# sd196821/QuadSim

Measured on AMD Instinct MI355X. Metric: env-steps/sec at N parallel envs (1/2/4/8 GPU); per-step state L2 err vs NumPy ref, higher is better.
Workload: dtype f32

## Files before the change

quadsim_amd/csrc/step_kernels.hpp:

```cpp
#pragma once

namespace {

#ifndef QS_BLOCK
#define QS_BLOCK 256
#endif
constexpr int kBlock = QS_BLOCK;
#ifndef QS_PREP_MAX_TILES
#define QS_PREP_MAX_TILES 1365
#endif
constexpr int64_t kPrepMaxTiles = QS_PREP_MAX_TILES;
#ifndef QS_SPLIT_MAX_ENVS
#define QS_SPLIT_MAX_ENVS 131072
#endif
constexpr int64_t kSplitMaxEnvs = QS_SPLIT_MAX_ENVS;

struct StepArgs {
    float *st;
    float *par;
    const float *actions;
    float *obs;
    float *reward;
    uint8_t *done;
    uint8_t *flags;
    float *term_obs;
    float *term_state;
    float *slab;
    int64_t n;
    int64_t tile0, tile_end;
    int64_t dbg_shift;
    int64_t io_env0, io_n;
    int64_t T;
    uint64_t step_idx;
    unsigned long long *ctr;
    uint64_t gid0;
    EnvConst C;
    RandCfg rc;
    Par par_nom;
    int auto_reset;
    int randomise;
    float nominal_obs[12];
    const float *init;
    unsigned *owner;
    unsigned *err;
    unsigned long long *stamps;
    unsigned long long stamp_cap, stamp_tiles;
};

__device__ __forceinline__ void load_env(const float *__restrict__ st, int64_t tile, int lane, Env &e)
{
    const float *b = st + tile * (int64_t)(kRecWords * kTile) + lane;
#pragma unroll
    for (int i = 0; i < 13; ++i) e.sc[i] = b[(F_SC + i) * kTile];
#pragma unroll
    for (int i = 0; i < 13; ++i) e.st[i] = b[(F_ST + i) * kTile];
#pragma unroll
    for (int i = 0; i < 4; ++i) e.uc[i] = b[(F_UC + i) * kTile];
#pragma unroll
    for (int i = 0; i < 4; ++i) e.ut[i] = b[(F_UT + i) * kTile];
#pragma unroll
    for (int i = 0; i < 4; ++i) e.qd[i] = b[(F_QD + i) * kTile];
    e.ls = b[F_LS * kTile];
    e.t = b[F_T * kTile];
}

__device__ __forceinline__ void load_env_or_nominal(const StepArgs &A, int64_t tile, int lane, bool active, Env &e)
{
    if (active) load_env(A.st, tile, lane, e);
    else { nominal_init(e.sc, e.st); for (int i = 0; i < 4; ++i) { e.uc[i] = 0.0f; e.ut[i] = 0.0f; e.qd[i] = i == 0; } e.ls = 0.0f; e.t = 0.0f; }
}

__device__ __forceinline__ void store_env(float *__restrict__ st, int64_t tile, int lane, const Env &e)
{
    float *b = st + tile * (int64_t)(kRecWords * kTile) + lane;
#pragma unroll
    for (int i = 0; i < 13; ++i) QS_ST(&b[(F_SC + i) * kTile], e.sc[i]);
#pragma unroll
    for (int i = 0; i < 13; ++i) QS_ST(&b[(F_ST + i) * kTile], e.st[i]);
#pragma unroll
    for (int i = 0; i < 4; ++i) QS_ST(&b[(F_UC + i) * kTile], e.uc[i]);
#pragma unroll
    for (int i = 0; i < 4; ++i) QS_ST(&b[(F_UT + i) * kTile], e.ut[i]);
#pragma unroll
    for (int i = 0; i < 4; ++i) QS_ST(&b[(F_QD + i) * kTile], e.qd[i]);
    QS_ST(&b[F_LS * kTile], e.ls);
    QS_ST(&b[F_T * kTile], e.t);
}

__device__ __forceinline__ Par load_par(const float *__restrict__ par, int64_t tile, int lane)
{
    const float *b = par + tile * (int64_t)(kParWords * kTile) + lane;
    Par P;
    P.m = b[0]; P.Ixx = b[kTile]; P.Iyy = b[2 * kTile]; P.Izz = b[3 * kTile];
    return P;
}

__device__ __forceinline__ void store_par(float *__restrict__ par, int64_t tile, int lane, const Par &P)
{
    float *b = par + tile * (int64_t)(kParWords * kTile) + lane;
    b[0] = P.m; b[kTile] = P.Ixx; b[2 * kTile] = P.Iyy; b[3 * kTile] = P.Izz;
}

struct TileLane { int lane; int64_t tile, env; bool active; };
__device__ __forceinline__ TileLane tile_lane(int64_t n)
{
    const int lane = threadIdx.x & (kTile - 1);
    const int64_t tile = (int64_t)blockIdx.x * (kBlock / kTile) + (threadIdx.x >> 6);
    const int64_t env = tile * kTile + lane;
    return {lane, tile, env, env < n};
}

__device__ __forceinline__ void store_obs(float *__restrict__ obs, int64_t env, const float o[12])
{
    typedef float f4 __attribute__((ext_vector_type(4)));
    f4 *p = reinterpret_cast<f4 *>(obs + env * 12);
    QS_SO(&p[0], (f4{o[0], o[1], o[2], o[3]}));
    QS_SO(&p[1], (f4{o[4], o[5], o[6], o[7]}));
    QS_SO(&p[2], (f4{o[8], o[9], o[10], o[11]}));
}

__device__ __forceinline__ void store_obs_cached(float *__restrict__ obs, int64_t env, const float o[12])
{
    float4 *p = reinterpret_cast<float4 *>(obs + env * 12);
    p[0] = make_float4(o[0], o[1], o[2], o[3]);
    p[1] = make_float4(o[4], o[5], o[6], o[7]);
    p[2] = make_float4(o[8], o[9], o[10], o[11]);
}

__device__ __forceinline__ uint64_t step_counter_begin(const StepArgs &A, int64_t tile) { return A.ctr[tile]; }
__device__ __forceinline__ uint64_t step_counter_begin_vmem(const StepArgs &A, int64_t tile)
{
    int zero;
    asm("v_mov_b32 %0, 0" : "=v"(zero));
    return A.ctr[tile + zero];
}
__device__ __forceinline__ void step_counter_end(const StepArgs &A, int64_t tile, int lane, uint64_t k)
{
    if (lane == 0) A.ctr[tile] = k + (uint64_t)A.T;
}

constexpr unsigned kUnowned = 0xffffffffu;
__device__ __forceinline__ unsigned chain_owner_request(const StepArgs &A, int64_t tile)
{
    const unsigned *p = A.owner ? A.owner + tile : reinterpret_cast<const unsigned *>(A.ctr + tile);
    const unsigned v = __hip_atomic_load(p, __ATOMIC_RELAXED, __HIP_MEMORY_SCOPE_AGENT);
    return A.owner ? v : kUnowned;
}

__device__ __forceinline__ bool chain_owner_mismatch(const StepArgs &A, int64_t tile, int lane, unsigned own)
{
    const unsigned xcc = __builtin_amdgcn_s_getreg((3 << 11) | (0 << 6) | 20) & 15u;
    if (own == kUnowned) {
        unsigned seen = kUnowned;
        if (lane == 0) {
            unsigned expect = kUnowned;
            __hip_atomic_compare_exchange_strong(&A.owner[tile], &expect, xcc, __ATOMIC_RELAXED, __ATOMIC_RELAXED, __HIP_MEMORY_SCOPE_AGENT);
            seen = expect;
        }
        own = __builtin_amdgcn_readfirstlane(seen);
        if (own == kUnowned) return false;
    }
    if (own != xcc) {
        if (lane == 0) __hip_atomic_fetch_or(A.err, 1u, __ATOMIC_RELAXED, __HIP_MEMORY_SCOPE_SYSTEM);
        return true;
    }
    return false;
}

__device__ __forceinline__ bool chain_tile_misplaced(const StepArgs &A, int64_t tile, int lane)
{
    if (!A.owner) return false;
    return chain_owner_mismatch(A, tile, lane, chain_owner_request(A, tile));
}

__device__ __forceinline__ int64_t launch_tile(const StepArgs &A, int64_t b)
{
    const int64_t nt = A.tile_end - A.tile0;
    b += A.dbg_shift;
    b -= (b >= nt) ? nt : 0;
    return A.tile0 + b;
}

template <bool PARAMS, int RMODE>
__device__ __forceinline__ void maybe_reset(Env &e, Par &P, const StepArgs &A, int64_t env, uint64_t k, float obs[12], unsigned flags,
                                            bool &done, bool write_term);

template <int INTEG, bool PARAMS, int RMODE>
__device__ __forceinline__ void step_and_maybe_reset(Env &e, Par &P, const float a[4], const StepArgs &A, int64_t env,
                                                     uint64_t k, float obs[12], float &reward, unsigned &flags,
                                                     bool &done, bool write_term)
{
    env_step<INTEG>(e, a, P, A.C, obs, reward, flags);
    maybe_reset<PARAMS, RMODE>(e, P, A, env, k, obs, flags, done, write_term);
}

template <bool PARAMS, int RMODE>
__device__ __forceinline__ void maybe_reset(Env &e, Par &P, const StepArgs &A, int64_t env, uint64_t k, float obs[12], unsigned flags,
                                            bool &done, bool write_term)
{
    done = (flags & (FLAG_OVERLIMIT | FLAG_OVERTIME)) != 0;
    if (done && A.auto_reset) {
        if (write_term && A.term_obs) store_obs(A.term_obs, env - A.io_env0, obs);
        if (write_term && A.term_state) {
            float *ts = A.term_state + (env - A.io_env0) * 26;
#pragma unroll
            for (int i = 0; i < 13; ++i) { ts[i] = e.sc[i]; ts[13 + i] = e.st[i]; }
        }
        if (RMODE == 0) {
            nominal_init(e.sc, e.st);
#pragma unroll
            for (int i = 0; i < 4; ++i) { e.uc[i] = 0.0f; e.ut[i] = 0.0f; }
            e.ls = 0.0f;
            e.t = 0.0f;
#pragma unroll
            for (int i = 0; i < 12; ++i) obs[i] = A.nominal_obs[i];
        } else if (RMODE == 3) {
            float ic[13], it[13];
            const float *src = A.init + env * 26;
#pragma unroll
            for (int i = 0; i < 13; ++i) { ic[i] = src[i]; it[i] = src[13 + i]; }
            env_reset<false>(e, ic, it, obs);
        } else {
            float ic[13], it[13];
            Par Pn;
            random_init<RMODE == 2>(A.rc, STREAM_AUTORESET, A.gid0 + (uint64_t)env, k + 1, ic, it, Pn);
            if (PARAMS && RMODE == 2) P = Pn;
            env_reset<true>(e, ic, it, obs);
        }
    }
}

template <int INTEG, bool PARAMS, int RMODE>
__global__ __launch_bounds__(kBlock) void k_env(StepArgs A)
{
    const int lane = threadIdx.x & (kTile - 1);
    const int64_t wg_tile = (int64_t)blockIdx.x * (kBlock / kTile) + (threadIdx.x >> 6);
    if (wg_tile >= A.tile_end - A.tile0) return;
    const int64_t tile = launch_tile(A, wg_tile);
    const int64_t env = tile * kTile + lane;
    if (env >= A.n) return;
    if (chain_tile_misplaced(A, tile, lane)) return;
    const int64_t io = env - A.io_env0;
    QS_ASSERT(io >= 0 && io < A.io_n);
    const uint64_t k0 = step_counter_begin_vmem(A, tile);
    float4 av_next = make_float4(0.0f, 0.0f, 0.0f, 0.0f);
    if (A.actions) av_next = reinterpret_cast<const float4 *>(A.actions)[io];
    Env e;
    load_env(A.st, tile, lane, e);
    Par P = A.par_nom;
    if (PARAMS) P = load_par(A.par, tile, lane);
#pragma clang loop unroll(disable)
    for (int64_t t = 0; t < A.T; ++t) {
        const uint64_t k = k0 + (uint64_t)t;
        const int64_t o = t * A.io_n + io;
        float a[4];
        if (A.actions) {
            const float4 av = av_next;
            if (t + 1 < A.T) av_next = reinterpret_cast<const float4 *>(A.actions)[o + A.io_n];
            a[0] = av.x; a[1] = av.y; a[2] = av.z; a[3] = av.w;
        } else {
            random_action(A.rc.seed, A.gid0 + (uint64_t)env, k, a);
        }
        float obs[12], reward;
        unsigned flags;
        bool done;
        step_and_maybe_reset<INTEG, PARAMS, RMODE>(e, P, a, A, env, k, obs, reward, flags, done, true);
        if (A.slab) {
            float2 *row = reinterpret_cast<float2 *>(A.slab + o * 14);
#pragma unroll
            for (int i = 0; i < 6; ++i) row[i] = make_float2(obs[2 * i], obs[2 * i + 1]);
            row[6] = make_float2(reward, done ? 1.0f : 0.0f);
        } else {
            store_obs(A.obs, o, obs);
            QS_SO(&A.reward[o], reward);
            QS_SO(&A.done[o], (uint8_t)(done ? 1 : 0));
        }
        if (A.flags) QS_SO(&A.flags[o], (uint8_t)flags);
    }
    store_env(A.st, tile, lane, e);
    if (PARAMS && RMODE == 2) store_par(A.par, tile, lane, P);
    step_counter_end(A, tile, lane, k0);
}

constexpr int split_waves(int rmode, int prep) { return (prep == 2 && (rmode == 1 || rmode == 2)) ? 3 : 2; }


constexpr bool split_prep(int rmode, int prep) { return split_waves(rmode, prep) == 3; }
constexpr bool split_draw(int rmode, int prep) { return (rmode == 1 || rmode == 2) && !split_prep(rmode, prep); }
template <int RMODE, int PREP>
struct SplitLds {
    float tgt[13][kTile];
    float rst[split_prep(RMODE, PREP) ? 29 : 0][kTile];
    uint4 phx[split_draw(RMODE, PREP) ? 2 : 0][2][kTile];
    unsigned char done[kTile], limt[kTile];
    __device__ __forceinline__ Par reset_par(int lane) const { return Par{rst[25][lane], rst[26][lane], rst[27][lane], rst[28][lane]}; }
};

__device__ __forceinline__ void chaser_load(const float *b, float sc[13], float uc[4], float &ls, float &tt)
{
#pragma unroll
    for (int i = 0; i < 13; ++i) sc[i] = b[(F_SC + i) * kTile];
#pragma unroll
    for (int i = 0; i < 4; ++i) uc[i] = b[(F_UC + i) * kTile];
    ls = b[F_LS * kTile];
    tt = b[F_T * kTile];
}

__device__ __forceinline__ void chaser_store(float *bw, const float sc[13], const float uc[4], float ls, float tt)
{
#pragma unroll
    for (int i = 0; i < 13; ++i) QS_ST(&bw[(F_SC + i) * kTile], sc[i]);
#pragma unroll
    for (int i = 0; i < 4; ++i) QS_ST(&bw[(F_UC + i) * kTile], uc[i]);
    QS_ST(&bw[F_LS * kTile], ls);
    QS_ST(&bw[F_T * kTile], tt);
}

template <int RMODE, int PREP>
__device__ __forceinline__ bool chaser_score(SplitLds<RMODE, PREP> &L, int lane, const float sc[13], const float a[4], float tt, float &ls,
                                             const EnvConst &C, int auto_reset, bool lim_c, float obs[12], float &reward,
                                             unsigned &flags, bool &done)
{
    float st[13];
#pragma unroll
    for (int i = 0; i < 13; ++i) st[i] = L.tgt[i][lane];
    const bool lim_t = L.limt[lane] != 0;
    rel_obs(sc, st, obs);
    score_step(obs, a, sc[2], tt, ls, C, lim_c, lim_t, reward, flags);
    done = (flags & (FLAG_OVERLIMIT | FLAG_OVERTIME)) != 0;
    const bool rs = done && auto_reset;
    L.done[lane] = rs ? 1 : 0;
    return rs;
}

__device__ __forceinline__ void store_term_half(float *term_state, bool active, int64_t io, int half, const float s[13])
{
    if (term_state && active) {
        float *ts = term_state + io * 26 + 13 * half;
#pragma unroll
        for (int i = 0; i < 13; ++i) ts[i] = s[i];
    }
}

template <bool PARAMS, int RMODE, int PREP>
__device__ __forceinline__ void chaser_reset(const SplitLds<RMODE, PREP> &L, const StepArgs &A, int64_t env, bool active, int lane, int64_t t,
                                             float sc[13], float uc[4], float &ls, float &tt, Par &P, float obs[12])
{
    float ic[13], it[13];
    if (RMODE == 0) {
        nominal_init(ic, it);
#pragma unroll
        for (int i = 0; i < 12; ++i) obs[i] = A.nominal_obs[i];
    } else if (RMODE == 3) {
        const float *src = A.init + (active ? env : 0) * 26;
#pragma unroll
        for (int i = 0; i < 13; ++i) { ic[i] = src[i]; it[i] = src[13 + i]; }
        rel_obs<false>(ic, it, obs);
    } else {
        if constexpr (split_prep(RMODE, PREP)) {
#pragma unroll
            for (int i = 0; i < 13; ++i) ic[i] = L.rst[i][lane];
#pragma unroll
            for (int i = 0; i < 12; ++i) obs[i] = L.rst[13 + i][lane];
            if (PARAMS && RMODE == 2) P = L.reset_par(lane);
        } else {
            const uint4 w0 = L.phx[t & 1][0][lane], w1 = RMODE == 2 ? L.phx[t & 1][1][lane] : make_uint4(0, 0, 0, 0);
            Par Pn;
            random_init_apply<RMODE == 2>(A.rc, w0, w1, ic, it, Pn);
            if (PARAMS && RMODE == 2) P = Pn;
            rel_obs<true>(ic, it, obs);
        }
    }
#pragma unroll
    for (int i = 0; i < 13; ++i) sc[i] = ic[i];
#pragma unroll
    for (int i = 0; i < 4; ++i) uc[i] = 0.0f;
    ls = 0.0f;
    tt = 0.0f;
}

__device__ __forceinline__ void target_load(const float *b, float st[13], float ut[4], float qd[4])
{
#pragma unroll
    for (int i = 0; i < 13; ++i) st[i] = b[(F_ST + i) * kTile];
#pragma unroll
    for (int i = 0; i < 4; ++i) ut[i] = b[(F_UT + i) * kTile];
#pragma unroll
    for (int i = 0; i < 4; ++i) qd[i] = b[(F_QD + i) * kTile];
}

__device__ __forceinline__ void target_store(float *bw, const float st[13], const float ut[4], const float qd[4])
{
#pragma unroll
    for (int i = 0; i < 13; ++i) QS_ST(&bw[(F_ST + i) * kTile], st[i]);
#pragma unroll
    for (int i = 0; i < 4; ++i) QS_ST(&bw[(F_UT + i) * kTile], ut[i]);
#pragma unroll
    for (int i = 0; i < 4; ++i) QS_ST(&bw[(F_QD + i) * kTile], qd[i]);
}

template <int RMODE, int PREP>
__device__ __forceinline__ void target_publish(SplitLds<RMODE, PREP> &L, const StepArgs &A, int64_t env, int lane, uint64_t k, int64_t t,
                                               const float st[13], bool lim_t, uint4 &w0, uint4 &w1)
{
#pragma unroll
    for (int i = 0; i < 13; ++i) L.tgt[i][lane] = st[i];
    L.limt[lane] = lim_t ? 1 : 0;
    w0 = make_uint4(0, 0, 0, 0);
    w1 = w0;
    if constexpr (split_draw(RMODE, PREP)) {
        random_init_words<RMODE == 2>(A.rc, STREAM_AUTORESET, A.gid0 + (uint64_t)env, k + 1, w0, w1);
        L.phx[t & 1][0][lane] = w0;
        if (RMODE == 2) L.phx[t & 1][1][lane] = w1;
    }
}

__device__ __forceinline__ void target_command(const EnvConst &C, float qd[4], const float pre[13], float m, float ut[4])
{
    const float pdes[3] = {10.0f, -50.0f, 5.0f};
    const float vdes[3] = {C.vdes_x, 0.0f, 0.0f};
    const float dv[3] = {0.0f, 0.0f, 0.0f};
    float u_t[4];
    target_control(C.kind, pdes, vdes, qd, 0.0f, pre, dv, m, u_t);
    u_limit(u_t, m * kG, ut);
}

template <bool PARAMS, int RMODE, int PREP>
__device__ __forceinline__ void target_reset(const SplitLds<RMODE, PREP> &L, const StepArgs &A, int64_t env, bool active, int lane,
                                             const uint4 &w0, const uint4 &w1, float st[13], float ut[4], Par &P)
{
    float ic[13], it[13];
    if (RMODE == 3) {
        const float *src = A.init + (active ? env : 0) * 26;
#pragma unroll
        for (int i = 0; i < 13; ++i) it[i] = src[13 + i];
    } else {
        nominal_init(ic, it);
        if (PARAMS && RMODE == 2) {
            if constexpr (split_prep(RMODE, PREP)) {
                P = L.reset_par(lane);
            } else {
                random_init_apply<true>(A.rc, w0, w1, ic, it, P);
                nominal_init(ic, it);
            }
        }
    }
#pragma unroll
    for (int i = 0; i < 13; ++i) st[i] = it[i];
#pragma unroll
    for (int i = 0; i < 4; ++i) ut[i] = 0.0f;
}

template <bool PARAMS, int RMODE, int PREP>
__device__ __forceinline__ void prep_publish(SplitLds<RMODE, PREP> &L, const RandCfg &rc, int lane, const uint4 &w0, const uint4 &w1)
{
    float ic[13], it_[13], robs[12];
    Par Pn;
    random_init_apply<RMODE == 2>(rc, w0, w1, ic, it_, Pn);
    rel_obs<true>(ic, it_, robs);
#pragma unroll
    for (int i = 0; i < 13; ++i) L.rst[i][lane] = ic[i];
#pragma unroll
    for (int i = 0; i < 12; ++i) L.rst[13 + i][lane] = robs[i];
    if (PARAMS && RMODE == 2) {
        L.rst[25][lane] = Pn.m; L.rst[26][lane] = Pn.Ixx; L.rst[27][lane] = Pn.Iyy; L.rst[28][lane] = Pn.Izz;
    }
}

constexpr int kResWords = 8;
constexpr unsigned long long kResPtrMask = (1ull << 48) - 1;
enum { RES_STEP = 0, RES_EXIT = 1, RES_IDLE = 2, RES_SKIP = 3 };
constexpr int kResWin = 32;
constexpr int kResWinSlots = 16;

struct ResArgs {
    const unsigned long long *ring;
    unsigned long long *rseq;
    unsigned *wcnt;
    unsigned *fin;
    unsigned long long *h_prog;
    unsigned long long *h_fin;
    unsigned long long seq0;
    unsigned long long base;
    unsigned long long stop_seq;
    unsigned long long slots_mask;
    unsigned long long idle_ticks;
    unsigned lane_tiles;
};

struct ResDesc {
    const float *actions;
    float *obs, *reward;
    uint8_t *done, *flags;
    float *term_obs, *term_state;
};

__device__ __forceinline__ unsigned long long res_request(const ResArgs &R, unsigned long long s, int lane)
{
    return __hip_atomic_load(R.ring + (s & R.slots_mask) * kResWords + (lane & 7), __ATOMIC_RELAXED, __HIP_MEMORY_SCOPE_SYSTEM);
}

__device__ __forceinline__ bool res_fresh(unsigned long long w, unsigned long long s, int lane)
{
    bool ok = (w >> 48) == (s & 0xffffull);
    if ((lane & 7) == 7) ok = ok && (unsigned)w == (unsigned)(s >> 16);
    return __all(ok);
}

__device__ __forceinline__ unsigned long long res_word(unsigned long long w, int i)
{
    const unsigned lo = (unsigned)__builtin_amdgcn_readlane((int)(unsigned)w, i);
    const unsigned hi = (unsigned)__builtin_amdgcn_readlane((int)(unsigned)(w >> 32), i);
    return (((unsigned long long)hi << 32) | lo) & kResPtrMask;
}

__device__ __forceinline__ int res_resolve(const ResArgs &R, unsigned long long s, int lane, unsigned long long w, ResDesc &D)
{
    if (!res_fresh(w, s, lane)) {
        const unsigned long long t0 = __builtin_amdgcn_s_memrealtime();
        for (;;) {
            __builtin_amdgcn_s_sleep(4);
            w = res_request(R, s, lane);
            if (res_fresh(w, s, lane)) break;
            if (__builtin_amdgcn_s_memrealtime() - t0 > R.idle_ticks) return RES_IDLE;
        }
    }
    D.actions = (const float *)res_word(w, 0);
    D.obs = (float *)res_word(w, 1);
    D.reward = (float *)res_word(w, 2);
    D.done = (uint8_t *)res_word(w, 3);
    D.flags = (uint8_t *)res_word(w, 4);
    D.term_obs = (float *)res_word(w, 5);
    D.term_state = (float *)res_word(w, 6);
    return ((res_word(w, 7) >> 32) & 0xff) == 0 ? RES_STEP : RES_EXIT;
}

__device__ __forceinline__ float4 res_action(const float *actions, int64_t io, int64_t io_n)
{
    typedef unsigned u4 __attribute__((ext_vector_type(4)));
    const __amdgpu_buffer_rsrc_t r = __builtin_amdgcn_make_buffer_rsrc((void *)actions, (short)0, (int)(io_n * 16), 0x00020000);
    const u4 v = __builtin_amdgcn_raw_buffer_load_b128(r, (int)(io * 16), 0, 17);
    return make_float4(__uint_as_float(v.x), __uint_as_float(v.y), __uint_as_float(v.z), __uint_as_float(v.w));
}

__device__ __forceinline__ unsigned res_report(const ResArgs &R, unsigned long long s, int64_t tile, int lane)
{
    const unsigned long long x = s - R.base + (unsigned long long)(tile % kResWin) + 1;
    if (x % kResWin != 0) return ~0u;
    unsigned old = 0;
    if (lane == 0) old = __hip_atomic_fetch_add(R.wcnt + (x / kResWin) % kResWinSlots, 1u, __ATOMIC_RELAXED, __HIP_MEMORY_SCOPE_AGENT);
    return old;
}

__device__ __forceinline__ void res_report_done(const ResArgs &R, unsigned old, unsigned long long s, int64_t tile, int lane)
{
    if (old == ~0u || lane != 0 || (old + 1) % R.lane_tiles != 0) return;
    const unsigned long long x = s - R.base + (unsigned long long)(tile % kResWin) + 1;
    __hip_atomic_store(R.h_prog, R.base + x - kResWin + 1, __ATOMIC_RELAXED, __HIP_MEMORY_SCOPE_SYSTEM);
}

template <int INTEG, bool PARAMS, int RMODE, int PREP>
__global__ __launch_bounds__(3 * kTile) void k_env_resident(StepArgs A, ResArgs R)
{
    __shared__ SplitLds<RMODE, PREP> L;
    __shared__ int s_cmd[2];
    __shared__ unsigned long long s_tsp[2];
    const int lane = threadIdx.x & (kTile - 1);
    const int role = threadIdx.x >> 6;
    const int64_t tile = launch_tile(A, blockIdx.x);
    const int64_t env = tile * kTile + lane;
    bool active = env < A.n;
    const int64_t io = env - A.io_env0;
    QS_ASSERT(tile < A.tile_end && (!active || (io >= 0 && io < A.io_n)));
    const uint64_t k0 = step_counter_begin_vmem(A, tile);
    unsigned long long seq = 0;
    int cmd = RES_STEP;
    ResDesc D{};
    {
        if (role == 0) {
            seq = R.seq0 ? R.seq0 : R.rseq[tile];
            seq = ((unsigned long long)__builtin_amdgcn_readfirstlane((int)(unsigned)(seq >> 32)) << 32) |
                  (unsigned)__builtin_amdgcn_readfirstlane((int)(unsigned)seq);
            cmd = seq >= R.stop_seq ? RES_SKIP : res_resolve(R, seq, lane, res_request(R, seq, lane), D);
            if (cmd == RES_STEP) res_report_done(R, res_report(R, seq, tile, lane), seq, tile, lane);
            if (lane == 0) { s_cmd[0] = cmd; s_tsp[0] = (unsigned long long)D.term_state; }
        }
        __syncthreads();
        cmd = s_cmd[0];
    }
    QS_STAMP_DECL;
    QS_STAMP_AT(0);
    const float *b = A.st + tile * (int64_t)(kRecWords * kTile) + lane;
    float *bw = A.st + tile * (int64_t)(kRecWords * kTile) + lane;
    Par P = A.par_nom;
    if (PARAMS) P = load_par(A.par, tile, lane);
    if (role == 0) {
        __builtin_amdgcn_s_setprio(3);
        float sc[13], uc[4], ls, tt;
        chaser_load(b, sc, uc, ls, tt);
        float4 av_next = make_float4(0.0f, 0.0f, 0.0f, 0.0f);
        if (cmd == RES_STEP && active) av_next = res_action(D.actions, io, A.io_n);
#if defined(QS_STAMP) && QS_STAMP + 0 < 2
        asm volatile("s_waitcnt vmcnt(1)" ::: "memory");
#endif
        QS_STAMP_AT(1);
        int64_t t = 0;
#pragma clang loop unroll(disable)
        for (; cmd == RES_STEP; ++t) {
            const int64_t o = io;
            const unsigned long long wn = res_request(R, seq + t + 1, lane);
            tt += 1.0f;
            const bool lim_c = drone_advance<INTEG>(sc, uc, P, A.C.dt);
            float a[4];
            ResDesc Dn{};
            unsigned rep = ~0u;
            const float4 av = av_next;
            const int cmdn = res_resolve(R, seq + t + 1, lane, wn, Dn);
            if (cmdn == RES_STEP) {
                if (active) av_next = res_action(Dn.actions, io, A.io_n);
                rep = res_report(R, seq + t + 1, tile, lane);
            }
            if (lane == 0) { s_cmd[(t + 1) & 1] = cmdn; s_tsp[(t + 1) & 1] = (unsigned long long)Dn.term_state; }
            a[0] = av.x; a[1] = av.y; a[2] = av.z; a[3] = av.w;
            float u_c[4];
            chaser_command(a, P.m, u_c);
            u_limit(u_c, P.m * kG, uc);
            QS_STAMP_AT(2);
            __syncthreads();
            QS_STAMP_AT(3);
            float obs[12], reward;
            unsigned flags;
            bool done;
            const bool rs = chaser_score(L, lane, sc, a, tt, ls, A.C, A.auto_reset, lim_c, obs, reward, flags, done);
            QS_STAMP_AT(4);
            __syncthreads();
            QS_STAMP_AT(5);
            if (rs) {
                if (D.term_obs && active) store_obs(D.term_obs, io, obs);
                store_term_half(D.term_state, active, io, 0, sc);
                chaser_reset<PARAMS>(L, A, env, active, lane, t, sc, uc, ls, tt, P, obs);
            }
            QS_STAMP_AT(6);
            if (active) {
                store_obs(D.obs, o, obs);
                QS_SO(&D.reward[o], reward);
                QS_SO(&D.done[o], (uint8_t)(done ? 1 : 0));
                if (D.flags) QS_SO(&D.flags[o], (uint8_t)flags);
            }
            res_report_done(R, rep, seq + t + 1, tile, lane);
            D = Dn;
            cmd = cmdn;
        }
        if (t > 0) {
            if (active) {
                chaser_store(bw, sc, uc, ls, tt);
                if (PARAMS && RMODE == 2) store_par(A.par, tile, lane, P);
            }
        }
        {
            if (cmd != RES_SKIP && lane == 0) {
                if (t > 0) A.ctr[tile] = k0 + (uint64_t)t;
                R.rseq[tile] = seq + (unsigned long long)t + (cmd == RES_EXIT ? 1 : 0);
                if (cmd == RES_EXIT) {
                    const unsigned old = __hip_atomic_fetch_add(R.fin, 1u, __ATOMIC_RELAXED, __HIP_MEMORY_SCOPE_AGENT);
                    if (old + 1 == R.lane_tiles)
                        __hip_atomic_store(R.h_fin, seq + (unsigned long long)t + 1, __ATOMIC_RELAXED, __HIP_MEMORY_SCOPE_SYSTEM);
                }
            }
        }
#if defined(QS_STAMP) && QS_STAMP + 0 < 2
        asm volatile("s_waitcnt vmcnt(0)" ::: "memory");
#endif
        QS_STAMP_AT(7);
        QS_STAMP_FLUSH();
    } else if (role == 1) {
        float st[13], ut[4], qd[4];
        target_load(b, st, ut, qd);
#if defined(QS_STAMP) && QS_STAMP + 0 < 2
        asm volatile("s_waitcnt vmcnt(0)" ::: "memory");
#endif
        QS_STAMP_AT(1);
        int64_t t = 0;
#pragma clang loop unroll(disable)
        for (; cmd == RES_STEP; ++t) {
            float pre[13];
#pragma unroll
            for (int i = 0; i < 13; ++i) pre[i] = st[i];
            const bool lim_t = drone_advance<INTEG>(st, ut, P, A.C.dt);
            uint4 w0, w1;
            target_publish(L, A, env, lane, k0 + (uint64_t)t, t, st, lim_t, w0, w1);
            QS_STAMP_AT(2);
            __syncthreads();
            QS_STAMP_AT(3);
            float *const term_state = (float *)s_tsp[t & 1];
            target_command(A.C, qd, pre, P.m, ut);
            QS_STAMP_AT(4);
            __syncthreads();
            QS_STAMP_AT(5);
            if (L.done[lane]) {
                store_term_half(term_state, active, io, 1, st);
                target_reset<PARAMS>(L, A, env, active, lane, w0, w1, st, ut, P);
            }
            cmd = s_cmd[(t + 1) & 1];
        }
        if (active && t > 0) target_store(bw, st, ut, qd);
        QS_STAMP_AT(6);
        QS_STAMP_FLUSH();
    } else if constexpr (split_prep(RMODE, PREP)) {
        int64_t t = 0;
#pragma clang loop unroll(disable)
        for (; cmd == RES_STEP; ++t) {
            uint4 w0, w1 = make_uint4(0, 0, 0, 0);
            random_init_words<RMODE == 2>(A.rc, STREAM_AUTORESET, A.gid0 + (uint64_t)env, k0 + (uint64_t)t + 1, w0, w1);
            __syncthreads();
            prep_publish<PARAMS>(L, A.rc, lane, w0, w1);
            __syncthreads();
            cmd = s_cmd[(t + 1) & 1];
        }
    }
}

template <int INTEG, bool PARAMS, int RMODE, int PREP>
__global__ __launch_bounds__(3 * kTile) void k_env_split(StepArgs A)
{
    __shared__ SplitLds<RMODE, PREP> L;
    const int lane = threadIdx.x & (kTile - 1);
    const int role = threadIdx.x >> 6;
    const int64_t tile = launch_tile(A, blockIdx.x);
    const int64_t env = tile * kTile + lane;
    bool active = env < A.n;
    const int64_t io = env - A.io_env0;
    QS_ASSERT(tile < A.tile_end && (!active || (io >= 0 && io < A.io_n)));
    const unsigned owner_xcc = chain_owner_request(A, tile);
    const uint64_t k0 = step_counter_begin_vmem(A, tile);
    QS_STAMP_DECL;
    QS_STAMP_AT(0);
    const float *b = A.st + tile * (int64_t)(kRecWords * kTile) + lane;
    float *bw = A.st + tile * (int64_t)(kRecWords * kTile) + lane;
    Par P = A.par_nom;
    if (PARAMS) P = load_par(A.par, tile, lane);
    if (role == 0) {
        if (A.T > 1) __builtin_amdgcn_s_setprio(3);
        float sc[13], uc[4], ls, tt;
        chaser_load(b, sc, uc, ls, tt);
        float4 av_next = make_float4(0.0f, 0.0f, 0.0f, 0.0f);
        if (A.actions && active) av_next = reinterpret_cast<const float4 *>(A.actions)[io];
#if defined(QS_STAMP) && QS_STAMP + 0 < 2
        asm volatile("s_waitcnt vmcnt(1)" ::: "memory");
#endif
        QS_STAMP_AT(1);
#pragma clang loop unroll(disable)
        for (int64_t t = 0; t < A.T; ++t) {
            const uint64_t k = k0 + (uint64_t)t;
            const int64_t o = t * A.io_n + io;
            tt += 1.0f;
            const bool lim_c = drone_advance<INTEG>(sc, uc, P, A.C.dt);
            if (A.owner && chain_owner_mismatch(A, tile, lane, owner_xcc)) active = false;
            float a[4];
            if (A.actions) {
                const float4 av = av_next;
                if (t + 1 < A.T && active) av_next = reinterpret_cast<const float4 *>(A.actions)[o + A.io_n];
                a[0] = av.x; a[1] = av.y; a[2] = av.z; a[3] = av.w;
            } else {
                random_action(A.rc.seed, A.gid0 + (uint64_t)env, k, a);
            }
            float u_c[4];
            chaser_command(a, P.m, u_c);
            u_limit(u_c, P.m * kG, uc);
            QS_STAMP_AT(2);
            __syncthreads();
            QS_STAMP_AT(3);
            if (A.T == 1) __builtin_amdgcn_s_setprio(3);
            float obs[12], reward;
            unsigned flags;
            bool done;
            const bool rs = chaser_score(L, lane, sc, a, tt, ls, A.C, A.auto_reset, lim_c, obs, reward, flags, done);
            QS_STAMP_AT(4);
            __syncthreads();
            QS_STAMP_AT(5);
            if (rs) {
                if (A.term_obs && active) store_obs(A.term_obs, io, obs);
                store_term_half(A.term_state, active, io, 0, sc);
                chaser_reset<PARAMS>(L, A, env, active, lane, t, sc, uc, ls, tt, P, obs);
            }
            QS_STAMP_AT(6);
            if (active) {
                if (A.slab) {
                    float2 *row = reinterpret_cast<float2 *>(A.slab + o * 14);
#pragma unroll
                    for (int i = 0; i < 6; ++i) row[i] = make_float2(obs[2 * i], obs[2 * i + 1]);
                    row[6] = make_float2(reward, done ? 1.0f : 0.0f);
                } else {
                    store_obs(A.obs, o, obs);
                    QS_SO(&A.reward[o], reward);
                    QS_SO(&A.done[o], (uint8_t)(done ? 1 : 0));
                }
                if (A.flags) QS_SO(&A.flags[o], (uint8_t)flags);
            }
        }
        if (active) {
            chaser_store(bw, sc, uc, ls, tt);
            if (PARAMS && RMODE == 2) store_par(A.par, tile, lane, P);
        }
        if (!A.owner || active || env >= A.n) step_counter_end(A, tile, lane, k0);
#if defined(QS_STAMP) && QS_STAMP + 0 < 2
        asm volatile("s_waitcnt vmcnt(0)" ::: "memory");
#endif
        QS_STAMP_AT(7);
        QS_STAMP_FLUSH();
    } else if (role == 1) {
        float st[13], ut[4], qd[4];
        target_load(b, st, ut, qd);
        if (A.T == 1) __builtin_amdgcn_s_setprio(3);
#if defined(QS_STAMP) && QS_STAMP + 0 < 2
        asm volatile("s_waitcnt vmcnt(0)" ::: "memory");
#endif
        QS_STAMP_AT(1);
#pragma clang loop unroll(disable)
        for (int64_t t = 0; t < A.T; ++t) {
            float pre[13];
#pragma unroll
            for (int i = 0; i < 13; ++i) pre[i] = st[i];
            const bool lim_t = drone_advance<INTEG>(st, ut, P, A.C.dt);
            if (A.owner && chain_owner_mismatch(A, tile, lane, owner_xcc)) active = false;
            uint4 w0, w1;
            target_publish(L, A, env, lane, k0 + (uint64_t)t, t, st, lim_t, w0, w1);
            QS_STAMP_AT(2);
            __syncthreads();
            QS_STAMP_AT(3);
            if (A.T == 1) __builtin_amdgcn_s_setprio(0);
            target_command(A.C, qd, pre, P.m, ut);
            QS_STAMP_AT(4);
            __syncthreads();
            QS_STAMP_AT(5);
            if (L.done[lane]) {
                store_term_half(A.term_state, active, io, 1, st);
                target_reset<PARAMS>(L, A, env, active, lane, w0, w1, st, ut, P);
            }
        }
        if (active) target_store(bw, st, ut, qd);
        QS_STAMP_AT(6);
        QS_STAMP_FLUSH();
    } else if constexpr (split_prep(RMODE, PREP)) {
#pragma clang loop unroll(disable)
        for (int64_t t = 0; t < A.T; ++t) {
            uint4 w0, w1 = make_uint4(0, 0, 0, 0);
            random_init_words<RMODE == 2>(A.rc, STREAM_AUTORESET, A.gid0 + (uint64_t)env, k0 + (uint64_t)t + 1, w0, w1);
            __syncthreads();
            prep_publish<PARAMS>(L, A.rc, lane, w0, w1);
            __syncthreads();
        }
    }
}

template <int INTEG, bool PARAMS>
__global__ __launch_bounds__(kBlock) void k_hover(StepArgs A)
{
    const int lane = threadIdx.x & (kTile - 1);
    const int64_t tile = A.tile0 + (int64_t)blockIdx.x * (kBlock / kTile) + (threadIdx.x >> 6);
    const int64_t env = tile * kTile + lane;
    if (tile >= A.tile_end || env >= A.n) return;
    const int64_t io = env - A.io_env0;
    QS_ASSERT(io >= 0 && io < A.io_n);
    const uint64_t k0 = step_counter_begin(A, tile);
    float *b = A.st + tile * (int64_t)(kRecWords * kTile) + lane;
    float s[13], up[4];
#pragma unroll
    for (int i = 0; i < 13; ++i) s[i] = b[(F_SC + i) * kTile];
#pragma unroll
    for (int i = 0; i < 4; ++i) up[i] = b[(F_UC + i) * kTile];
    Par P = A.par_nom;
    if (PARAMS) P = load_par(A.par, tile, lane);
#pragma clang loop unroll(disable)
    for (int64_t t = 0; t < A.T; ++t) {
        const int64_t o = t * A.io_n + io;
        float a[4];
        if (A.actions) {
            const float4 av = reinterpret_cast<const float4 *>(A.actions)[o];
            a[0] = av.x; a[1] = av.y; a[2] = av.z; a[3] = av.w;
        } else {
            random_action(A.rc.seed, A.gid0 + (uint64_t)env, k0 + (uint64_t)t, a);
#pragma unroll
            for (int i = 0; i < 4; ++i) a[i] = 0.5f * a[i] + 0.5f;
        }
        float reward;
        unsigned flags;
        hover_step<INTEG>(s, up, a, P, A.C.dt, reward, flags);
        const bool done = (flags & FLAG_OVERLIMIT) != 0;
        if (done && A.auto_reset) {
            if (A.term_obs) for (int i = 0; i < 13; ++i) A.term_obs[io * 13 + i] = s[i];
            const float *src = A.init + env * 13;
#pragma unroll
            for (int i = 0; i < 13; ++i) s[i] = src[i];
#pragma unroll
            for (int i = 0; i < 4; ++i) up[i] = 0.0f;
        }
#pragma unroll
        for (int i = 0; i < 13; ++i) A.obs[o * 13 + i] = s[i];
        A.reward[o] = reward;
        A.done[o] = done ? 1 : 0;
        if (A.flags) A.flags[o] = (uint8_t)flags;
    }
#pragma unroll
    for (int i = 0; i < 13; ++i) b[(F_SC + i) * kTile] = s[i];
#pragma unroll
    for (int i = 0; i < 4; ++i) b[(F_UC + i) * kTile] = up[i];
    step_counter_end(A, tile, lane, k0);
}

__global__ __launch_bounds__(kBlock) void k_ctor_init(float *init, int64_t n, int hover, uint64_t seed, uint64_t gid0)
{
    const int64_t env = (int64_t)blockIdx.x * kBlock + threadIdx.x;
    if (env >= n) return;
    uint4 w = philox_block(seed, STREAM_CTOR, gid0 + (uint64_t)env, 0);
    if (!hover) {
        float *d = init + env * 26;
        for (int i = 0; i < 26; ++i) d[i] = 0.0f;
        d[0] = __fmaf_rn(sym(u16lo(w.x)), 0.3f, 8.0f);
        d[1] = __fmaf_rn(sym(u16hi(w.x)), 0.3f, -50.0f);
        d[2] = __fmaf_rn(sym(u16lo(w.y)), 0.3f, 5.0f);
        d[6] = 1.0f;
        d[13] = 10.0f; d[14] = -50.0f; d[15] = 5.0f; d[19] = 1.0f;
    } else {
        float *d = init + env * 13;
        for (int i = 0; i < 13; ++i) d[i] = 0.0f;
        d[0] = sym(u16lo(w.x));
        d[1] = sym(u16hi(w.x));
        d[2] = __fmaf_rn(sym(u16lo(w.y)), 1.0f, 5.0f);
        float e0 = sym(u16hi(w.y)) * 0.2f, e1 = sym(u16lo(w.z)) * 0.2f, e2 = sym(u16hi(w.z)) * 0.2f;
        float sr, cr, sp, cp, sy, cy;
        q_sincos_small(0.5f * e0, sr, cr);
        q_sincos_small(0.5f * e1, sp, cp);
        q_sincos_small(0.5f * e2, sy, cy);
        euler2quat_trig(sr, cr, sp, cp, sy, cy, d + 6);
    }
}

__global__ __launch_bounds__(kBlock) void k_fill_init_nominal(float *init, int64_t n)
{
    const int64_t env = (int64_t)blockIdx.x * kBlock + threadIdx.x;
    if (env >= n) return;
    float sc[13], st[13];
    nominal_init(sc, st);
    for (int i = 0; i < 13; ++i) { init[env * 26 + i] = sc[i]; init[env * 26 + 13 + i] = st[i]; }
}

__global__ __launch_bounds__(kBlock) void k_reset(StepArgs A, const uint8_t *__restrict__ mask, int init_all)
{
    const int lane = threadIdx.x & (kTile - 1);
    const int64_t tile = (int64_t)blockIdx.x * (kBlock / kTile) + (threadIdx.x >> 6);
    const int64_t env = tile * kTile + lane;
    if (env >= A.n) return;
    if (mask && !mask[env]) return;
    Env e;
    load_env(A.st, tile, lane, e);
    float ic[13], it[13], obs[12];
    if (A.init) {
        const float *src = A.init + env * 26;
        for (int i = 0; i < 13; ++i) { ic[i] = src[i]; it[i] = src[13 + i]; }
    } else if (A.randomise) {
        Par Pn;
        random_init<true>(A.rc, STREAM_RESET, A.gid0 + (uint64_t)env, A.ctr[tile], ic, it, Pn);
        if (A.randomise >= 2) store_par(A.par, tile, lane, Pn);
    } else {
        nominal_init(ic, it);
    }
    if (init_all) { e.qd[0] = 1.0f; e.qd[1] = 0.0f; e.qd[2] = 0.0f; e.qd[3] = 0.0f; }
    env_reset(e, ic, it, obs);
    store_env(A.st, tile, lane, e);
    if (A.obs) store_obs(A.obs, env, obs);
}

__global__ __launch_bounds__(kBlock) void k_hover_reset(StepArgs A, const uint8_t *__restrict__ mask)
{
    const int lane = threadIdx.x & (kTile - 1);
    const int64_t tile = (int64_t)blockIdx.x * (kBlock / kTile) + (threadIdx.x >> 6);
    const int64_t env = tile * kTile + lane;
    if (env >= A.n) return;
    if (mask && !mask[env]) return;
    float *b = A.st + tile * (int64_t)(kRecWords * kTile) + lane;
    const float *src = A.init + env * 13;
    for (int i = 0; i < 13; ++i) { b[(F_SC + i) * kTile] = src[i]; if (A.obs) A.obs[env * 13 + i] = src[i]; }
    for (int i = 0; i < 4; ++i) b[(F_UC + i) * kTile] = 0.0f;
}

__global__ __launch_bounds__(kBlock) void k_fill_ctr(unsigned long long *ctr, int64_t tiles, unsigned long long k)
{
    const int64_t i = (int64_t)blockIdx.x * kBlock + threadIdx.x;
    if (i < tiles) ctr[i] = k;
}

__global__ void k_nominal_obs(float *out)
{
    float sc[13], st[13], o[12];
    nominal_init(sc, st);
    rel_obs(sc, st, o);
    for (int i = 0; i < 12; ++i) out[i] = o[i];
}

__global__ __launch_bounds__(kBlock) void k_fill_par(float *par, int64_t n, Par P)
{
    const int lane = threadIdx.x & (kTile - 1);
    const int64_t tile = (int64_t)blockIdx.x * (kBlock / kTile) + (threadIdx.x >> 6);
    if (tile * kTile + lane >= n) return;
    store_par(par, tile, lane, P);
}

__global__ __launch_bounds__(kBlock) void k_fill_actions(float *__restrict__ actions, int64_t n, int64_t T, uint64_t seed,
                                                         uint64_t gid0, uint64_t step0)
{
    const int64_t i = (int64_t)blockIdx.x * kBlock + threadIdx.x;
    if (i >= n * T) return;
    const int64_t t = i / n, env = i - t * n;
    float a[4];
    random_action(seed, gid0 + (uint64_t)env, step0 + (uint64_t)t, a);
    reinterpret_cast<float4 *>(actions)[i] = make_float4(a[0], a[1], a[2], a[3]);
}

struct StateIO {
    float *chaser, *target, *u_prev, *qdes, *ls, *t;
};
template <bool TO_USER>
__global__ __launch_bounds__(kBlock) void k_state_io(float *st, int64_t n, StateIO io)
{
    const int lane = threadIdx.x & (kTile - 1);
    const int64_t tile = (int64_t)blockIdx.x * (kBlock / kTile) + (threadIdx.x >> 6);
    const int64_t env = tile * kTile + lane;
    if (env >= n) return;
    float *b = st + tile * (int64_t)(kRecWords * kTile) + lane;
    auto mv = [&](float *user, int f) {
        if (!user) return;
        if (TO_USER) *user = b[f * kTile];
        else b[f * kTile] = *user;
    };
    for (int i = 0; i < 13; ++i) mv(io.chaser ? io.chaser + env * 13 + i : nullptr, F_SC + i);
    for (int i = 0; i < 13; ++i) mv(io.target ? io.target + env * 13 + i : nullptr, F_ST + i);
    for (int i = 0; i < 8; ++i) mv(io.u_prev ? io.u_prev + env * 8 + i : nullptr, F_UC + i);
    for (int i = 0; i < 4; ++i) mv(io.qdes ? io.qdes + env * 4 + i : nullptr, F_QD + i);
    mv(io.ls ? io.ls + env : nullptr, F_LS);
    mv(io.t ? io.t + env : nullptr, F_T);
}

template <bool TO_USER>
__global__ __launch_bounds__(kBlock) void k_par_io(float *par, int64_t n, float *mass, float *inertia)
{
    const int lane = threadIdx.x & (kTile - 1);
    const int64_t tile = (int64_t)blockIdx.x * (kBlock / kTile) + (threadIdx.x >> 6);
    const int64_t env = tile * kTile + lane;
    if (env >= n) return;
    float *b = par + tile * (int64_t)(kParWords * kTile) + lane;
    if (TO_USER) {
        if (mass) mass[env] = b[0];
        if (inertia) for (int i = 0; i < 3; ++i) inertia[env * 3 + i] = b[(1 + i) * kTile];
    } else {
        if (mass) b[0] = mass[env];
        if (inertia) for (int i = 0; i < 3; ++i) b[(1 + i) * kTile] = inertia[env * 3 + i];
    }
}

inline int64_t tiles_of(int64_t n) { return (n + kTile - 1) / kTile; }
inline unsigned grid_tiles(int64_t n) { return (unsigned)((tiles_of(n) + (kBlock / kTile) - 1) / (kBlock / kTile)); }
inline unsigned grid_flat(int64_t n) { return (unsigned)((n + kBlock - 1) / kBlock); }

}
```

Measured before the change: 26.89 billion.

## Move resident-kernel descriptor polling to prep wavefront and share via LDS slot

When a separate prep wavefront exists, it now polls the host ring for the next step's descriptor and publishes the decoded pointers and command through an LDS slot. The chaser wavefront no longer sits on the critical path waiting for the host. Pointers are cast to the global address space so the compiler can emit global rather than flat memory ops. The change adds LDS traffic and readlanes, and because the chaser now issues its action load only after the barrier, that load may have less time to complete.

```diff
diff --git a/quadsim_amd/csrc/step_kernels.hpp b/quadsim_amd/csrc/step_kernels.hpp
--- a/quadsim_amd/csrc/step_kernels.hpp
+++ b/quadsim_amd/csrc/step_kernels.hpp
@@ -507,6 +507,12 @@
     return __all(ok);
 }
 
+template <class T>
+__device__ __forceinline__ T *res_ptr(unsigned long long a)
+{
+    return (T *)(__attribute__((address_space(1))) T *)a;
+}
+
 __device__ __forceinline__ unsigned long long res_word(unsigned long long w, int i)
 {
     const unsigned lo = (unsigned)__builtin_amdgcn_readlane((int)(unsigned)w, i);
@@ -514,7 +520,7 @@
     return (((unsigned long long)hi << 32) | lo) & kResPtrMask;
 }
 
-__device__ __forceinline__ int res_resolve(const ResArgs &R, unsigned long long s, int lane, unsigned long long w, ResDesc &D)
+__device__ __forceinline__ bool res_poll(const ResArgs &R, unsigned long long s, int lane, unsigned long long &w)
 {
     if (!res_fresh(w, s, lane)) {
         const unsigned long long t0 = __builtin_amdgcn_s_memrealtime();
@@ -522,17 +528,50 @@
             __builtin_amdgcn_s_sleep(4);
             w = res_request(R, s, lane);
             if (res_fresh(w, s, lane)) break;
-            if (__builtin_amdgcn_s_memrealtime() - t0 > R.idle_ticks) return RES_IDLE;
-        }
-    }
-    D.actions = (const float *)res_word(w, 0);
-    D.obs = (float *)res_word(w, 1);
-    D.reward = (float *)res_word(w, 2);
-    D.done = (uint8_t *)res_word(w, 3);
-    D.flags = (uint8_t *)res_word(w, 4);
-    D.term_obs = (float *)res_word(w, 5);
-    D.term_state = (float *)res_word(w, 6);
-    return ((res_word(w, 7) >> 32) & 0xff) == 0 ? RES_STEP : RES_EXIT;
+            if (__builtin_amdgcn_s_memrealtime() - t0 > R.idle_ticks) return false;
+        }
+    }
+    return true;
+}
+
+__device__ __forceinline__ int res_command(unsigned long long w) { return ((res_word(w, 7) >> 32) & 0xff) == 0 ? RES_STEP : RES_EXIT; }
+
+__device__ __forceinline__ int res_decode(unsigned long long w, ResDesc &D)
+{
+    D.actions = res_ptr<const float>(res_word(w, 0));
+    D.obs = res_ptr<float>(res_word(w, 1));
+    D.reward = res_ptr<float>(res_word(w, 2));
+    D.done = res_ptr<uint8_t>(res_word(w, 3));
+    D.flags = res_ptr<uint8_t>(res_word(w, 4));
+    D.term_obs = res_ptr<float>(res_word(w, 5));
+    D.term_state = res_ptr<float>(res_word(w, 6));
+    return res_command(w);
+}
+
+typedef unsigned long long ResSlot[kResWords];
+
+__device__ __forceinline__ void res_hand_over(ResSlot &slot, int lane, unsigned long long w, int cmd)
+{
+    if (lane < kResWords) slot[lane] = lane == kResWords - 1 ? (unsigned long long)cmd : (w & kResPtrMask);
+}
+
+__device__ __forceinline__ unsigned long long res_slot_word(unsigned long long w, int i)
+{
+    return ((unsigned long long)(unsigned)__builtin_amdgcn_readlane((int)(unsigned)(w >> 32), i) << 32) |
+           (unsigned)__builtin_amdgcn_readlane((int)(unsigned)w, i);
+}
+
+__device__ __forceinline__ int res_take(const ResSlot &slot, int lane, ResDesc &D)
+{
+    const unsigned long long w = slot[lane & (kResWords - 1)];
+    D.actions = res_ptr<const float>(res_slot_word(w, 0));
+    D.obs = res_ptr<float>(res_slot_word(w, 1));
+    D.reward = res_ptr<float>(res_slot_word(w, 2));
+    D.done = res_ptr<uint8_t>(res_slot_word(w, 3));
+    D.flags = res_ptr<uint8_t>(res_slot_word(w, 4));
+    D.term_obs = res_ptr<float>(res_slot_word(w, 5));
+    D.term_state = res_ptr<float>(res_slot_word(w, 6));
+    return __builtin_amdgcn_readlane((int)(unsigned)w, 7);
 }
 
 __device__ __forceinline__ float4 res_action(const float *actions, int64_t io, int64_t io_n)
@@ -552,6 +591,16 @@
     return old;
 }
 
+__device__ __forceinline__ void res_leave(const ResArgs &R, unsigned long long next, int cmd, int64_t tile, int lane)
+{
+    if (cmd == RES_SKIP || lane != 0) return;
+    R.rseq[tile] = next + (cmd == RES_EXIT ? 1 : 0);
+    if (cmd == RES_EXIT) {
+        const unsigned old = __hip_atomic_fetch_add(R.fin, 1u, __ATOMIC_RELAXED, __HIP_MEMORY_SCOPE_AGENT);
+        if (old + 1 == R.lane_tiles) __hip_atomic_store(R.h_fin, next + 1, __ATOMIC_RELAXED, __HIP_MEMORY_SCOPE_SYSTEM);
+    }
+}
+
 __device__ __forceinline__ void res_report_done(const ResArgs &R, unsigned old, unsigned long long s, int64_t tile, int lane)
 {
     if (old == ~0u || lane != 0 || (old + 1) % R.lane_tiles != 0) return;
@@ -559,12 +608,14 @@
     __hip_atomic_store(R.h_prog, R.base + x - kResWin + 1, __ATOMIC_RELAXED, __HIP_MEMORY_SCOPE_SYSTEM);
 }
 
+constexpr int res_owner(int rmode, int prep) { return split_prep(rmode, prep) ? 2 : 0; }
+
 template <int INTEG, bool PARAMS, int RMODE, int PREP>
 __global__ __launch_bounds__(3 * kTile) void k_env_resident(StepArgs A, ResArgs R)
 {
     __shared__ SplitLds<RMODE, PREP> L;
-    __shared__ int s_cmd[2];
-    __shared__ unsigned long long s_tsp[2];
+    __shared__ ResSlot s_desc[2];
+    constexpr int OWNER = res_owner(RMODE, PREP);
     const int lane = threadIdx.x & (kTile - 1);
     const int role = threadIdx.x >> 6;
     const int64_t tile = launch_tile(A, blockIdx.x);
@@ -577,16 +628,21 @@
     int cmd = RES_STEP;
     ResDesc D{};
     {
-        if (role == 0) {
+        if (role == OWNER) {
             seq = R.seq0 ? R.seq0 : R.rseq[tile];
             seq = ((unsigned long long)__builtin_amdgcn_readfirstlane((int)(unsigned)(seq >> 32)) << 32) |
                   (unsigned)__builtin_amdgcn_readfirstlane((int)(unsigned)seq);
-            cmd = seq >= R.stop_seq ? RES_SKIP : res_resolve(R, seq, lane, res_request(R, seq, lane), D);
+            unsigned long long w = 0;
+            cmd = RES_SKIP;
+            if (seq < R.stop_seq) {
+                w = res_request(R, seq, lane);
+                cmd = res_poll(R, seq, lane, w) ? res_command(w) : RES_IDLE;
+            }
             if (cmd == RES_STEP) res_report_done(R, res_report(R, seq, tile, lane), seq, tile, lane);
-            if (lane == 0) { s_cmd[0] = cmd; s_tsp[0] = (unsigned long long)D.term_state; }
+            res_hand_over(s_desc[0], lane, w, cmd);
         }
         __syncthreads();
-        cmd = s_cmd[0];
+        cmd = res_take(s_desc[0], lane, D);
     }
     QS_STAMP_DECL;
     QS_STAMP_AT(0);
@@ -604,23 +660,28 @@
         asm volatile("s_waitcnt vmcnt(1)" ::: "memory");
 #endif
         QS_STAMP_AT(1);
+        asm volatile("" :: "v"(av_next.x), "v"(av_next.y), "v"(av_next.z), "v"(av_next.w));
         int64_t t = 0;
 #pragma clang loop unroll(disable)
         for (; cmd == RES_STEP; ++t) {
             const int64_t o = io;
-            const unsigned long long wn = res_request(R, seq + t + 1, lane);
+            unsigned long long wn = 0;
+            if constexpr (OWNER == 0) wn = res_request(R, seq + t + 1, lane);
             tt += 1.0f;
             const bool lim_c = drone_advance<INTEG>(sc, uc, P, A.C.dt);
             float a[4];
             ResDesc Dn{};
             unsigned rep = ~0u;
+            int cmdn = RES_IDLE;
             const float4 av = av_next;
-            const int cmdn = res_resolve(R, seq + t + 1, lane, wn, Dn);
-            if (cmdn == RES_STEP) {
-                if (active) av_next = res_action(Dn.actions, io, A.io_n);
-                rep = res_report(R, seq + t + 1, tile, lane);
+            if constexpr (OWNER == 0) {
+                if (res_poll(R, seq + t + 1, lane, wn)) cmdn = res_decode(wn, Dn);
+                if (cmdn == RES_STEP) {
+                    if (active) av_next = res_action(Dn.actions, io, A.io_n);
+                    rep = res_report(R, seq + t + 1, tile, lane);
+                }
+                res_hand_over(s_desc[(t + 1) & 1], lane, wn, cmdn);
             }
-            if (lane == 0) { s_cmd[(t + 1) & 1] = cmdn; s_tsp[(t + 1) & 1] = (unsigned long long)Dn.term_state; }
             a[0] = av.x; a[1] = av.y; a[2] = av.z; a[3] = av.w;
             float u_c[4];
             chaser_command(a, P.m, u_c);
@@ -628,6 +689,10 @@
             QS_STAMP_AT(2);
             __syncthreads();
             QS_STAMP_AT(3);
+            if constexpr (OWNER != 0) {
+                cmdn = res_take(s_desc[(t + 1) & 1], lane, Dn);
+                if (cmdn == RES_STEP && active) av_next = res_action(Dn.actions, io, A.io_n);
+            }
             float obs[12], reward;
             unsigned flags;
             bool done;
@@ -635,6 +700,7 @@
             QS_STAMP_AT(4);
             __syncthreads();
             QS_STAMP_AT(5);
+            asm volatile("" :: "v"(av_next.x), "v"(av_next.y), "v"(av_next.z), "v"(av_next.w));
             if (rs) {
                 if (D.term_obs && active) store_obs(D.term_obs, io, obs);
                 store_term_half(D.term_state, active, io, 0, sc);
@@ -647,7 +713,7 @@
                 QS_SO(&D.done[o], (uint8_t)(done ? 1 : 0));
                 if (D.flags) QS_SO(&D.flags[o], (uint8_t)flags);
             }
-            res_report_done(R, rep, seq + t + 1, tile, lane);
+            if constexpr (OWNER == 0) res_report_done(R, rep, seq + t + 1, tile, lane);
             D = Dn;
             cmd = cmdn;
         }
@@ -656,18 +722,9 @@
                 chaser_store(bw, sc, uc, ls, tt);
                 if (PARAMS && RMODE == 2) store_par(A.par, tile, lane, P);
             }
-        }
-        {
-            if (cmd != RES_SKIP && lane == 0) {
-                if (t > 0) A.ctr[tile] = k0 + (uint64_t)t;
-                R.rseq[tile] = seq + (unsigned long long)t + (cmd == RES_EXIT ? 1 : 0);
-                if (cmd == RES_EXIT) {
-                    const unsigned old = __hip_atomic_fetch_add(R.fin, 1u, __ATOMIC_RELAXED, __HIP_MEMORY_SCOPE_AGENT);
-                    if (old + 1 == R.lane_tiles)
-                        __hip_atomic_store(R.h_fin, seq + (unsigned long long)t + 1, __ATOMIC_RELAXED, __HIP_MEMORY_SCOPE_SYSTEM);
-                }
-            }
-        }
+            if (lane == 0) A.ctr[tile] = k0 + (uint64_t)t;
+        }
+        if constexpr (OWNER == 0) res_leave(R, seq + (unsigned long long)t, cmd, tile, lane);
 #if defined(QS_STAMP) && QS_STAMP + 0 < 2
         asm volatile("s_waitcnt vmcnt(0)" ::: "memory");
 #endif
@@ -692,31 +749,43 @@
             QS_STAMP_AT(2);
             __syncthreads();
             QS_STAMP_AT(3);
-            float *const term_state = (float *)s_tsp[t & 1];
+            ResDesc Dn{};
+            const int cmdn = res_take(s_desc[(t + 1) & 1], lane, Dn);
             target_command(A.C, qd, pre, P.m, ut);
+            asm volatile("" :: "v"(qd[0]), "v"(qd[1]), "v"(qd[2]), "v"(qd[3]), "v"(ut[0]), "v"(ut[1]), "v"(ut[2]), "v"(ut[3]));
             QS_STAMP_AT(4);
             __syncthreads();
             QS_STAMP_AT(5);
             if (L.done[lane]) {
-                store_term_half(term_state, active, io, 1, st);
+                store_term_half(D.term_state, active, io, 1, st);
                 target_reset<PARAMS>(L, A, env, active, lane, w0, w1, st, ut, P);
             }
-            cmd = s_cmd[(t + 1) & 1];
+            D = Dn;
+            cmd = cmdn;
         }
         if (active && t > 0) target_store(bw, st, ut, qd);
         QS_STAMP_AT(6);
         QS_STAMP_FLUSH();
-    } else if constexpr (split_prep(RMODE, PREP)) {
+    } else if constexpr (OWNER == 2) {
         int64_t t = 0;
 #pragma clang loop unroll(disable)
         for (; cmd == RES_STEP; ++t) {
+            unsigned long long wn = res_request(R, seq + t + 1, lane);
             uint4 w0, w1 = make_uint4(0, 0, 0, 0);
             random_init_words<RMODE == 2>(A.rc, STREAM_AUTORESET, A.gid0 + (uint64_t)env, k0 + (uint64_t)t + 1, w0, w1);
+            int cmdn = RES_IDLE;
+            unsigned rep = ~0u;
+            if (res_poll(R, seq + t + 1, lane, wn)) cmdn = res_command(wn);
+            if (cmdn == RES_STEP) rep = res_report(R, seq + t + 1, tile, lane);
+            res_hand_over(s_desc[(t + 1) & 1], lane, wn, cmdn);
             __syncthreads();
+            asm volatile("" : "+v"(w0.x), "+v"(w0.y), "+v"(w0.z), "+v"(w0.w), "+v"(w1.x), "+v"(w1.y), "+v"(w1.z), "+v"(w1.w));
             prep_publish<PARAMS>(L, A.rc, lane, w0, w1);
             __syncthreads();
-            cmd = s_cmd[(t + 1) & 1];
-        }
+            res_report_done(R, rep, seq + t + 1, tile, lane);
+            cmd = cmdn;
+        }
+        res_leave(R, seq + (unsigned long long)t, cmd, tile, lane);
     }
 }
 
```

New measurement: 27.91 billion, median of 5. +3.8%, better.
